# KrisKennaway/ii-vision

Hardware: AMD Instinct MI355X
Metric: DHGR frames transcoded/sec (higher is better)
Workload: dtype u16; 1 GPU; DHGR NTSC palette 560x192 S-iid synthetic clips, 750 frames each, 14336 independent clips per GPU, Movie.encode control flow (490 opcodes/frame, bank flip per 2 KiB); palette=NTSC, streams_per_gpu=14336, greedy_form=shared, resident_clip_frames=750, opcodes_per_frame=490, parallelism=1 GPU x 14336 independent streams, no collective

## Files before the change

### ii-vision_amd/csrc/iiv_prologue.hip

```cpp
#include "iiv_host.h"
#include "iiv_edit.h"
#include "iiv_stream.h"
#include "iiv_wave.h"

namespace iiv {


constexpr int kProThreads = 1024;

__device__ static inline void lds_barrier()
{
    asm volatile("s_waitcnt lgkmcnt(0)\n\ts_barrier" ::: "memory");
}

#ifdef IIV_STAMPS
#define IIV_STAMP(i)                                                        \
    do {                                                                    \
        __syncthreads();                                                    \
        if (threadIdx.x == 0) S.stamps[i] = __builtin_amdgcn_s_memtime();   \
    } while (0)
#else
#define IIV_STAMP(i) do { } while (0)
#endif

__device__ static inline void cmpx(unsigned long long &lo, unsigned long long &hi, bool asc)
{
    bool sw = (lo > hi) == asc;
    unsigned long long t = lo;
    lo = sw ? hi : lo;
    hi = sw ? t : hi;
}

template <int KPT, int NT>
__device__ static inline void bitonic_sort(unsigned long long (&v)[KPT], unsigned long long *xbuf, int tid)
{
    constexpr int N = KPT * NT;
#pragma unroll
    for (int k = 2; k <= KPT; k <<= 1) {
#pragma unroll
        for (int j = k >> 1; j >= 1; j >>= 1) {
#pragma unroll
            for (int r = 0; r < KPT; r++)
                if ((r & j) == 0) cmpx(v[r], v[r | j], (((KPT * tid + r) & k) == 0));
        }
    }
    for (int k = 2 * KPT; k <= N; k <<= 1) {
        const bool asc = ((KPT * tid) & k) == 0;
        for (int j = k >> 1; j >= KPT; j >>= 1) {
            const int d = j / KPT;
            const bool take_min = ((tid & d) == 0) == asc;
            if (d < 64) {
#pragma unroll
                for (int r = 0; r < KPT; r++) {
                    unsigned long long p = __shfl_xor(v[r], d, 64);
                    v[r] = take_min ? (p < v[r] ? p : v[r]) : (p > v[r] ? p : v[r]);
                }
            } else {
#pragma unroll
                for (int r = 0; r < KPT; r++) xbuf[r * NT + tid] = v[r];
                __syncthreads();
#pragma unroll
                for (int r = 0; r < KPT; r++) {
                    unsigned long long p = xbuf[r * NT + (tid ^ d)];
                    v[r] = take_min ? (p < v[r] ? p : v[r]) : (p > v[r] ? p : v[r]);
                }
                __syncthreads();
            }
        }
#pragma unroll
        for (int j = KPT >> 1; j >= 1; j >>= 1) {
#pragma unroll
            for (int r = 0; r < KPT; r++)
                if ((r & j) == 0) cmpx(v[r], v[r | j], asc);
        }
    }
}

template <int KPT> __device__ static inline void write_order(uint32_t *order, const unsigned long long (&v)[KPT], int tid)
{
    uint32_t o[KPT];
#pragma unroll
    for (int j = 0; j < KPT; j++) o[j] = ((uint32_t)(v[j] >> 8) & 0x1fffu) | (((uint32_t)v[j] & 0xffu) << 16);
    if (KPT == 2) {
        *reinterpret_cast<uint2 *>(order + 2 * tid) = make_uint2(o[0], o[1]);
    } else {
        uint4 *q = reinterpret_cast<uint4 *>(order + KPT * tid);
#pragma unroll
        for (int j = 0; j < KPT / 4; j++) q[j] = make_uint4(o[4 * j], o[4 * j + 1], o[4 * j + 2], o[4 * j + 3]);
    }
}

__device__ static inline int wave_scan_incl(int v)
{
    v += __builtin_amdgcn_update_dpp(0, v, 0x111, 0xf, 0xf, false);
    v += __builtin_amdgcn_update_dpp(0, v, 0x112, 0xf, 0xf, false);
    v += __builtin_amdgcn_update_dpp(0, v, 0x114, 0xf, 0xf, false);
    v += __builtin_amdgcn_update_dpp(0, v, 0x118, 0xf, 0xf, false);
    v += __builtin_amdgcn_update_dpp(0, v, 0x142, 0xa, 0xf, false);
    v += __builtin_amdgcn_update_dpp(0, v, 0x143, 0xc, 0xf, false);
    return v;
}

template <int NT> __device__ static inline int block_scan_excl(int v, int tid, uint32_t *wsum, int &total)
{
    static_assert(NT == 1024, "sixteen waves: their totals are scanned in one DPP row");
    const int incl = wave_scan_incl(v);
    lds_barrier();
    if ((tid & 63) == 63) wsum[tid >> 6] = (uint32_t)incl;
    lds_barrier();
    int x = (int)wsum[tid & 15];
    x += __builtin_amdgcn_update_dpp(0, x, 0x111, 0xf, 0xf, false);
    x += __builtin_amdgcn_update_dpp(0, x, 0x112, 0xf, 0xf, false);
    x += __builtin_amdgcn_update_dpp(0, x, 0x114, 0xf, 0xf, false);
    x += __builtin_amdgcn_update_dpp(0, x, 0x118, 0xf, 0xf, false);
    const int w = __builtin_amdgcn_readfirstlane(tid >> 6);
    total = __builtin_amdgcn_readlane(x, 15);
    const int wbase = w ? __builtin_amdgcn_readlane(x, w - 1) : 0;
    return wbase + incl - v;
}

template <int NT> __device__ static inline int block_scan_excl_and_max(int v, int m, int tid, uint32_t *wsum, uint32_t *wmax, int &total, int &maxv)
{
    static_assert(NT == 1024, "sixteen waves");
    auto mx = [](int a, int b) { return a > b ? a : b; };
    const int incl = wave_scan_incl(v);
    m = mx(m, __builtin_amdgcn_update_dpp(0, m, 0xB1, 0xf, 0xf, false));
    m = mx(m, __builtin_amdgcn_update_dpp(0, m, 0x4E, 0xf, 0xf, false));
    m = mx(m, __builtin_amdgcn_update_dpp(0, m, 0x141, 0xf, 0xf, false));
    m = mx(m, __builtin_amdgcn_update_dpp(0, m, 0x140, 0xf, 0xf, false));
    m = mx(m, __builtin_amdgcn_update_dpp(0, m, 0x142, 0xf, 0xf, false));
    m = mx(m, __builtin_amdgcn_update_dpp(0, m, 0x143, 0xf, 0xf, false));
    lds_barrier();
    if ((tid & 63) == 63) {
        wsum[tid >> 6] = (uint32_t)incl;
        wmax[tid >> 6] = (uint32_t)m;
    }
    lds_barrier();
    int x = (int)wsum[tid & 15], y = (int)wmax[tid & 15];
    x += __builtin_amdgcn_update_dpp(0, x, 0x111, 0xf, 0xf, false);
    x += __builtin_amdgcn_update_dpp(0, x, 0x112, 0xf, 0xf, false);
    x += __builtin_amdgcn_update_dpp(0, x, 0x114, 0xf, 0xf, false);
    x += __builtin_amdgcn_update_dpp(0, x, 0x118, 0xf, 0xf, false);
    y = mx(y, __builtin_amdgcn_update_dpp(0, y, 0xB1, 0xf, 0xf, false));
    y = mx(y, __builtin_amdgcn_update_dpp(0, y, 0x4E, 0xf, 0xf, false));
    y = mx(y, __builtin_amdgcn_update_dpp(0, y, 0x141, 0xf, 0xf, false));
    y = mx(y, __builtin_amdgcn_update_dpp(0, y, 0x140, 0xf, 0xf, false));
    const int w = __builtin_amdgcn_readfirstlane(tid >> 6);
    total = __builtin_amdgcn_readlane(x, 15);
    maxv = __builtin_amdgcn_readfirstlane(y);
    const int wbase = w ? __builtin_amdgcn_readlane(x, w - 1) : 0;
    return wbase + incl - v;
}

template <int NT> __device__ static inline int block_max(int v, int tid, uint32_t *wsum)
{
    static_assert(NT == 1024, "sixteen waves");
    auto mx = [](int a, int b) { return a > b ? a : b; };
    v = mx(v, __builtin_amdgcn_update_dpp(0, v, 0xB1, 0xf, 0xf, false));
    v = mx(v, __builtin_amdgcn_update_dpp(0, v, 0x4E, 0xf, 0xf, false));
    v = mx(v, __builtin_amdgcn_update_dpp(0, v, 0x141, 0xf, 0xf, false));
    v = mx(v, __builtin_amdgcn_update_dpp(0, v, 0x140, 0xf, 0xf, false));
    v = mx(v, __builtin_amdgcn_update_dpp(0, v, 0x142, 0xf, 0xf, false));
    v = mx(v, __builtin_amdgcn_update_dpp(0, v, 0x143, 0xf, 0xf, false));
    lds_barrier();
    if ((tid & 63) == 63) wsum[tid >> 6] = (uint32_t)v;
    lds_barrier();
    int x = (int)wsum[tid & 15];
    x = mx(x, __builtin_amdgcn_update_dpp(0, x, 0xB1, 0xf, 0xf, false));
    x = mx(x, __builtin_amdgcn_update_dpp(0, x, 0x4E, 0xf, 0xf, false));
    x = mx(x, __builtin_amdgcn_update_dpp(0, x, 0x141, 0xf, 0xf, false));
    x = mx(x, __builtin_amdgcn_update_dpp(0, x, 0x140, 0xf, 0xf, false));
    return __builtin_amdgcn_readfirstlane(x);
}

__device__ static inline bool any_half_is_big(const uint32_t (&w)[4])
{
    typedef unsigned short u16x2 __attribute__((ext_vector_type(2)));
    const u16x2 a = __builtin_elementwise_max(__builtin_bit_cast(u16x2, w[0]), __builtin_bit_cast(u16x2, w[1]));
    const u16x2 b = __builtin_elementwise_max(__builtin_bit_cast(u16x2, w[2]), __builtin_bit_cast(u16x2, w[3]));
    const uint32_t m = __builtin_bit_cast(uint32_t, __builtin_elementwise_max(a, b));
    return m >= 0xffff0000u || (m & 0xffffu) == kUpBig;
}

template <int MODE, int DP>
__device__ __forceinline__ void prologue_body(StreamState *__restrict__ states, const uint8_t *__restrict__ frames_main,
                                              const uint8_t *__restrict__ frames_aux, int n_frames, const LaunchSeg &seg,
                                              const uint16_t *__restrict__ table, const ulonglong2 *__restrict__ strings,
                                              const uint16_t *__restrict__ sub, const uint32_t *__restrict__ dwl,
                                              const uint32_t *__restrict__ dwr, const uint32_t *__restrict__ hgr_dots,
                                              const uint32_t *__restrict__ dw_pieces)
{
    const int need = __builtin_amdgcn_readfirstlane(seg.need);
    if (need < 0) return;
    const int frame = __builtin_amdgcn_readfirstlane(seg.frame), is_aux = __builtin_amdgcn_readfirstlane(seg.is_aux);
    constexpr int BITS = ModeTraits<MODE>::kBits;
    constexpr int NB = ModeTraits<MODE>::kBanks;
    __shared__ __attribute__((aligned(16))) unsigned char lds[9728 + 65536];
    uint32_t *aux4k = reinterpret_cast<uint32_t *>(lds + 512);
    uint32_t(*mtb)[624] = reinterpret_cast<uint32_t(*)[624]>(lds + 4608);
    uint32_t *wsum = reinterpret_cast<uint32_t *>(lds + 9600);
    int &flag_bad = *reinterpret_cast<int *>(lds + 9664);
    int &sel_bucket = *reinterpret_cast<int *>(lds + 9668);
    int &sel_count = *reinterpret_cast<int *>(lds + 9672);
    int &big_bucket = *reinterpret_cast<int *>(lds + 9676);
    unsigned char *smem = lds + 9728;
    unsigned long long *keys = reinterpret_cast<unsigned long long *>(smem);
    uint32_t *gen = reinterpret_cast<uint32_t *>(smem + 32768);

    const int tid = threadIdx.x;
    StreamState &S = states[blockIdx.x];
    const size_t fbase = ((size_t)blockIdx.x * n_frames + frame) * 8192;

    IIV_STAMP(0);
    const int first = S.mt_np_idx;
    const int error_in = S.error;
    if (tid == 0) flag_bad = 0;
    uint32_t *gtab = reinterpret_cast<uint32_t *>(smem);
    uint32_t *hdot = aux4k;
    if (DP == IIV_DW_RECURRENCE) {
        reinterpret_cast<uint4 *>(gtab)[tid] = reinterpret_cast<const uint4 *>(dw_pieces + (MODE == kDHGR ? 4096 * is_aux : 0))[tid];
        if (MODE == kHGR) {
            constexpr int kRest = (int)kHgrPieceWords / 4 - kProThreads;
            static_assert(kRest > 0 && kRest <= kProThreads && kHgrPieceWords * 4 <= 32768, "the HGR pair-term table ends below the generated MT19937 blocks");
            if (tid < kRest) reinterpret_cast<uint4 *>(gtab)[kProThreads + tid] = reinterpret_cast<const uint4 *>(dw_pieces)[kProThreads + tid];
            if (tid >= kProThreads - kHgrDotLutEntries / 4) {
                const int q = tid - (kProThreads - kHgrDotLutEntries / 4);
                reinterpret_cast<uint4 *>(hdot)[q] = reinterpret_cast<const uint4 *>(hgr_dots)[q];
            }
        }
    }
    IIV_STAMP(10);
    for (int i = tid; i < 624; i += kProThreads) mtb[0][i] = S.mt_np[i];
    IIV_STAMP(11);
    __syncthreads();
    IIV_STAMP(1);
    const int own_b = (MODE == kDHGR && is_aux) ? 1 : 0;
    const int tgt_first = tid == 0 ? (int)((own_b ? frames_aux : frames_main) + fbase)[0] : 0;
    const int i0 = tid * 8;
    const bool mt_wave = tid >= kProThreads - 64;
    uint16_t *dwx = reinterpret_cast<uint16_t *>(mtb[1]);

    int32_t upv[8];
    {
        const uint4 a = *reinterpret_cast<const uint4 *>(S.up16[is_aux] + i0);
        const uint32_t w[4] = {a.x, a.y, a.z, a.w};
#pragma unroll
        for (int j = 0; j < 4; j++) {
            upv[2 * j] = (int32_t)(w[j] & 0xffffu);
            upv[2 * j + 1] = (int32_t)(w[j] >> 16);
        }
        if (any_half_is_big(w)) {
#pragma unroll
            for (int j = 0; j < 8; j++)
                if ((uint32_t)upv[j] == kUpBig) upv[j] = S.up[is_aux][i0 + j];
        }
    }
    if (mt_wave) {
        __builtin_amdgcn_s_setprio(3);
        const uint32_t *src = mtb[0];
#ifndef IIV_EXP_MT_BLOCKS
#define IIV_EXP_MT_BLOCKS 13
#endif
        const int n_blocks = __builtin_amdgcn_readfirstlane((first + 7679) / 624);
        const int nb = n_blocks < IIV_EXP_MT_BLOCKS ? n_blocks : IIV_EXP_MT_BLOCKS;
#ifndef IIV_HGR_MT_REGISTERS
#define IIV_HGR_MT_REGISTERS 1
#endif
        if (MODE == kDHGR || IIV_HGR_MT_REGISTERS) {
            mt_generate_wave(src, gen, nb, tid & 63);
        } else {
            for (int k = 0; k < nb; k++) {
                mt_twist_wave(src, gen + k * 624, tid & 63);
                src = gen + k * 624;
            }
        }
        __builtin_amdgcn_s_setprio(0);
    }
    IIV_STAMP(12);

    auto diff_weight = [&](uint32_t cm, uint32_t tm, int y) -> uint32_t {
        const int odd = y & 1;
        const int o = byte_offset<MODE>(y, is_aux);
        if (DP == IIV_DW_TABLE) return table[((size_t)o << (2 * BITS)) + ((size_t)cm << BITS) + tm];
        if (DP == IIV_DW_SPLIT) {
            using T = SplitTraits<MODE>;
            const uint32_t l = dwl[((((uint32_t)o << T::kLeftRowBits) + split_row_left<MODE>(cm, odd)) << T::kLeftRowBits) +
                                   split_row_left<MODE>(tm, odd)];
            const uint32_t r = dwr[((((uint32_t)o << T::kRightRowBits) + split_row_right<MODE>(cm, odd)) << T::kRightRowBits) +
                                   split_row_right<MODE>(tm, odd)];
            return combine(l, r);
        }
        if constexpr (MODE == kDHGR) {
            return 0u;
        } else {
            return hgr_dw_pieces_sum(hdot, reinterpret_cast<const unsigned char *>(gtab), cm, tm, odd);
        }
    };

    uint32_t dwv[8], tmv[8];
    uint32_t cpk[2] = {0, 0};
    int bad = 0;
    {
        const bool hole = is_hole(i0 & 255);
        const bool proxy = hole && !mt_wave;
        int grp = tid;
        if (proxy) {
            const int k = tid >> 4;
            grp = 960 + k + k / 15;
        }
        const int yb = (grp * 8) & 255;
#pragma unroll
        for (int j = 0; j < 8; j++) tmv[j] = dwv[j] = 0;
        const int oth_b = NB - 1 - own_b;
        const uint8_t *cur_own_g = S.mem[own_b] + grp * 8, *cur_oth_g = S.mem[oth_b] + grp * 8;
        const uint8_t *tgt_own_g = (own_b ? frames_aux : frames_main) + fbase + grp * 8;
        const uint8_t *tgt_oth_g = (oth_b ? frames_aux : frames_main) + fbase + grp * 8;
        unsigned long long own8[2], prv8[2], nxt8[2];
#pragma unroll
        for (int k = 0; k < 2; k++) {
            const uint8_t *own = k ? tgt_own_g : cur_own_g, *oth = k ? tgt_oth_g : cur_oth_g;
            own8[k] = *reinterpret_cast<const unsigned long long *>(own);
            if (MODE != kDHGR) {
                const unsigned long long before = yb > 0 ? own[-1] : 0, after = yb + 8 < 256 ? own[8] : 0;
                prv8[k] = (own8[k] << 8) | before;
                nxt8[k] = (own8[k] >> 8) | (after << 56);
                continue;
            }
            const unsigned long long o8 = *reinterpret_cast<const unsigned long long *>(oth);
            if (is_aux) {
                const unsigned long long before = yb > 0 ? oth[-1] : 0;
                prv8[k] = (o8 << 8) | before;
                nxt8[k] = o8;
            } else {
                const unsigned long long after = yb + 8 < 256 ? oth[8] : 0;
                prv8[k] = o8;
                nxt8[k] = (o8 >> 8) | (after << 56);
            }
        }
        if (hole) {
            const unsigned long long mine = proxy ? *reinterpret_cast<const unsigned long long *>(S.mem[own_b] + i0) : own8[0];
            if (mine) bad = kErrHoles;
        }
        if (!proxy) {
            cpk[0] = (uint32_t)own8[1];
            cpk[1] = (uint32_t)(own8[1] >> 32);
        }
        auto dw_pieces_sum = [&](uint32_t W, int parity) -> uint32_t {
            uint32_t acc = 0;
#pragma unroll
            for (int i = 0; i < 5; i++) {
                const uint32_t cur6 = __builtin_amdgcn_ubfe(W, 16 + 2 * i, 6);
                const uint32_t tgt6x4 = (i == 0 ? W << 2 : i == 1 ? W : W >> (2 * i - 2)) & 0xfcu;
                const uint32_t v = *reinterpret_cast<const uint32_t *>(reinterpret_cast<const unsigned char *>(gtab) + ((cur6 << 8) | tgt6x4));
                acc += ((i + parity) & 1) ? v >> 16 : v & 0xffffu;
            }
            return acc - 5u * kDwPieceBias;
        };
        if (!hole || proxy) {
#pragma unroll
            for (int j = 0; j < 8; j++) {
                const int jj = j & 3;
                const uint32_t sel = 0x0c000c00u | (uint32_t)jj | ((uint32_t)(4 + jj) << 16);
                auto pick = [&](const unsigned long long (&v)[2]) -> uint32_t {
                    const uint32_t c = j < 4 ? (uint32_t)v[0] : (uint32_t)(v[0] >> 32), t = j < 4 ? (uint32_t)v[1] : (uint32_t)(v[1] >> 32);
                    return __builtin_amdgcn_perm(c, t, sel);
                };
                const uint32_t pb = pick(prv8), ob = pick(own8), nb = pick(nxt8);
                if constexpr (MODE == kDHGR) {
                    const uint32_t W = ((pb >> 3) & 0x000e000eu) | ((ob & 0x007f007fu) << 4) | ((nb & 0x00070007u) << 11);
                    if (!proxy) tmv[j] = (W >> 1) & 0x1fffu;
                    if (!mt_wave) {
                        uint32_t d;
                        if (DP == IIV_DW_RECURRENCE) d = dw_pieces_sum(W, j & 1);
                        else d = diff_weight(W >> 17, (W >> 1) & 0x1fffu, yb + j);
                        if (proxy) dwx[(grp - 960) * 8 + j] = (uint16_t)d;
                        else dwv[j] = d;
                    }
                } else {
                    const uint32_t mid = (j & 1) ? ((ob & 0x007f007fu) << 4) | ((ob & 0x00800080u) >> 4) : ob << 3;
                    const uint32_t W = ((pb >> 5) & 0x00070007u) | mid | ((nb & 0x00030003u) << 12) | ((nb & 0x00800080u) << 4);
                    if (!proxy) tmv[j] = W & 0x3fffu;
                    if (!mt_wave) {
                        const uint32_t d = diff_weight(W >> 16, W & 0x3fffu, yb + j);
                        if (proxy) dwx[(grp - 960) * 8 + j] = (uint16_t)d;
                        else dwv[j] = d;
                    }
                }
            }
        }
    }
    uint32_t nzmask = 0;
    auto finish_bytes = [&]() {
#pragma unroll
        for (int j = 0; j < 8; j++) {
            int32_t u = upv[j];
            if (dwv[j] == 0) u = 0;
            u += (int32_t)dwv[j];
            if (u < 0) bad = kErrNegative;
            upv[j] = u;
            if (u != 0) nzmask |= 1u << j;
        }
        uint32_t pk[4];
#pragma unroll
        for (int j = 0; j < 4; j++) {
            typedef unsigned short u16x2 __attribute__((ext_vector_type(2)));
            const u16x2 c = __builtin_amdgcn_cvt_pk_u16((uint32_t)upv[2 * j], (uint32_t)upv[2 * j + 1]);
            pk[j] = __builtin_bit_cast(uint32_t, c);
        }
        *reinterpret_cast<uint4 *>(S.up16[is_aux] + i0) = make_uint4(pk[0], pk[1], pk[2], pk[3]);
        if (any_half_is_big(pk)) {
#pragma unroll
            for (int j = 0; j < 8; j++)
                if ((uint32_t)upv[j] >= kUpBig) S.up[is_aux][i0 + j] = upv[j];
        }
        uint4 *q = reinterpret_cast<uint4 *>(S.wd + i0);
        uint32_t wv[8];
#pragma unroll
        for (int j = 0; j < 8; j++)
            wv[j] = wd_word(split_row_left<MODE>(tmv[j], j & 1), split_row_right<MODE>(tmv[j], j & 1), dwv[j]);
        q[0] = make_uint4(wv[0], wv[1], wv[2], wv[3]);
        q[1] = make_uint4(wv[4], wv[5], wv[6], wv[7]);
        reinterpret_cast<uint8_t *>(S.nzbits)[tid] = (uint8_t)nzmask;
    };
    constexpr bool kFinishEarly = true;
    if (error_in) return;
    if (kFinishEarly && !mt_wave) finish_bytes();
    __builtin_amdgcn_s_setprio(3);
    lds_barrier();
    if (mt_wave && !is_hole(i0 & 255)) {
#pragma unroll
        for (int j = 0; j < 8; j++) dwv[j] = dwx[(tid - (kProThreads - 64)) * 8 + j];
    }
    if (!kFinishEarly || mt_wave) finish_bytes();
    if (tid < 256) S.pdone[tid] = 0;
    if (bad) flag_bad = bad;

    IIV_STAMP(2);
    uint32_t *hist = aux4k;
    uint32_t *wmax = reinterpret_cast<uint32_t *>(mtb[1]);
    uint16_t *start = reinterpret_cast<uint16_t *>(mtb[1]) + 64;
    int n, sh;
    int mx = 0;
#pragma unroll
    for (int j = 0; j < 8; j++) mx = upv[j] > mx ? upv[j] : mx;
    hist[tid] = 0;
    const int rank0 = block_scan_excl_and_max<kProThreads>(__popc(nzmask), mx, tid, wsum, wmax, n, mx);
    sh = mx < 1024 ? 0 : (32 - __clz(mx)) - 10;
    if (tid == 0) {
        sel_bucket = 0;
        sel_count = n;
        big_bucket = 0;
    }
#pragma unroll
    for (int j = 0; j < 8; j++)
        if (nzmask & (1u << j)) atomicAdd(&hist[upv[j] >> sh], 1u);
    lds_barrier();
    const int bcount = (int)hist[1023 - tid];
    int total_unused;
    const int bstart = block_scan_excl<kProThreads>(bcount, tid, wsum, total_unused);
    const bool want_prefix = need > 0 && need <= kSelNeedMax && n > need;
    if (want_prefix && bstart < need && bstart + bcount >= need) {
        sel_bucket = 1023 - tid;
        sel_count = bstart + bcount;
    }
    lds_barrier();
    const int n_sel = sel_count;
    const int first_bucket = sel_bucket;
    if (bcount > kBucketMax && (1023 - tid) >= first_bucket) big_bucket = 1;
    uint32_t selmask = 0;
#pragma unroll
    for (int j = 0; j < 8; j++)
        if ((nzmask & (1u << j)) && (upv[j] >> sh) >= first_bucket) selmask |= 1u << j;
    lds_barrier();
    const bool by_buckets = big_bucket == 0;
    uint32_t *cursor = aux4k;
    cursor[1023 - tid] = (uint32_t)bstart;
    start[1023 - tid] = (uint16_t)bstart;

    IIV_STAMP(3);
    if (!flag_bad) {
        const int blk = first + n > 0 ? (first + n - 1) / 624 : 0;
        const uint32_t *fin = blk ? gen + (blk - 1) * 624 : mtb[0];
        for (int w = tid; w < 624; w += kProThreads) S.mt_np[w] = fin[w];
        if (tid == 0) {
            S.mt_np_idx = first + n - blk * 624;
            S.draws_np += (unsigned long long)n;
        }
    }

    IIV_STAMP(4);
    unsigned long long kv[8];
    {
        int bk = (first + rank0) / 624, bw = first + rank0 - bk * 624;
#pragma unroll
        for (int j = 0; j < 8; j++) {
            kv[j] = ~0ull;
            if (nzmask & (1u << j)) {
                if (selmask & (1u << j)) {
                    const uint32_t nonce = mt_temper((bk ? gen + (bk - 1) * 624 : mtb[0])[bw]) & 0xffu;
                    kv[j] = ((unsigned long long)(0x7fffffffu - (uint32_t)upv[j]) << 29) |
                            ((unsigned long long)nonce << 21) | ((unsigned long long)(i0 + j) << 8) |
                            (unsigned long long)((cpk[j >> 2] >> (8 * (j & 3))) & 0xffu);
                }
                if (++bw == 624) {
                    bw = 0;
                    bk++;
                }
            }
        }
    }
    IIV_STAMP(5);
    if (by_buckets) {
        lds_barrier();
        IIV_STAMP(8);
        uint32_t slot[8];
#pragma unroll
        for (int j = 0; j < 8; j++) {
            slot[j] = 0;
            if (kv[j] != ~0ull) slot[j] = atomicAdd(&cursor[(0x7fffffffu - (uint32_t)(kv[j] >> 29)) >> sh], 1u);
        }
#pragma unroll
        for (int j = 0; j < 8; j++)
            if (kv[j] != ~0ull) keys[slot[j]] = kv[j];
        lds_barrier();
        IIV_STAMP(9);
        for (int t = tid; t < n_sel; t += kProThreads) {
            const unsigned long long key = keys[t];
            const int bk = (int)((0x7fffffffu - (uint32_t)(key >> 29)) >> sh);
            const int s0 = (int)start[bk];
            const int e0 = bk == 0 ? n : (int)start[bk - 1];
            const int last = e0 - 1;
            int below = 0;
            int i = s0;
            for (; i + 16 <= e0; i += 16) {
                unsigned long long kk[16];
#pragma unroll
                for (int u = 0; u < 16; u++) kk[u] = keys[i + u];
#pragma unroll
                for (int u = 0; u < 16; u++) below += kk[u] < key ? 1 : 0;
            }
            for (; i < e0; i += 4) {
                const unsigned long long k0 = keys[i];
                const unsigned long long k1 = keys[i + 1 < e0 ? i + 1 : last];
                const unsigned long long k2 = keys[i + 2 < e0 ? i + 2 : last];
                const unsigned long long k3 = keys[i + 3 < e0 ? i + 3 : last];
                below += (k0 < key ? 1 : 0) + ((i + 1 < e0 && k1 < key) ? 1 : 0) +
                         ((i + 2 < e0 && k2 < key) ? 1 : 0) + ((i + 3 < e0 && k3 < key) ? 1 : 0);
            }
            S.order[s0 + below] = ((uint32_t)(key >> 8) & 0x1fffu) | (((uint32_t)key & 0xffu) << 16);
        }
    } else if (n_sel <= 4 * kProThreads) {
        __syncthreads();
        int tot;
        int nsel_mine = 0;
#pragma unroll
        for (int j = 0; j < 8; j++) nsel_mine += kv[j] != ~0ull ? 1 : 0;
        int pos = block_scan_excl<kProThreads>(nsel_mine, tid, wsum, tot);
        const bool small = tot <= 2 * kProThreads;
        const int n_pad = small ? 2 * kProThreads : 4 * kProThreads;
        for (int i = tot + tid; i < n_pad; i += kProThreads) keys[i] = ~0ull;
#pragma unroll
        for (int j = 0; j < 8; j++)
            if (kv[j] != ~0ull) keys[pos++] = kv[j];
        __syncthreads();
        if (small) {
            unsigned long long v2[2] = {keys[2 * tid], keys[2 * tid + 1]};
            __syncthreads();
            bitonic_sort<2, kProThreads>(v2, keys, tid);
            write_order<2>(S.order, v2, tid);
        } else {
            unsigned long long v4[4] = {keys[4 * tid], keys[4 * tid + 1], keys[4 * tid + 2], keys[4 * tid + 3]};
            __syncthreads();
            bitonic_sort<4, kProThreads>(v4, keys, tid);
            write_order<4>(S.order, v4, tid);
        }
    } else {
        __syncthreads();
        bitonic_sort<8, kProThreads>(kv, keys, tid);
        write_order<8>(S.order, kv, tid);
    }
    IIV_STAMP(6);
    IIV_STAMP(7);
    if (tid == 0) {
        S.n_sorted = n_sel;
        S.truncated = n_sel < n ? 1 : 0;
        S.head = 0;
        S.n_pushed = 0;
        S.exhausted = 0;
        S.gen_active = 1;
        S.gen_is_aux = is_aux;
        S.gen_frame = frame;
        S.pad_content = tgt_first;
        if (flag_bad && S.error == 0) S.error = flag_bad;
    }
}

template <int MODE, int DP>
__global__ __launch_bounds__(kProThreads, 8) void prologue_kernel(StreamState *__restrict__ states,
                                                               const uint8_t *__restrict__ frames_main,
                                                               const uint8_t *__restrict__ frames_aux, int n_frames,
                                                               const LaunchSeg *__restrict__ segs, int seg_stride,
                                                               const uint16_t *__restrict__ table,
                                                               const ulonglong2 *__restrict__ strings,
                                                               const uint16_t *__restrict__ sub,
                                                               const uint32_t *__restrict__ dwl,
                                                               const uint32_t *__restrict__ dwr,
                                                               const uint32_t *__restrict__ hgr_dots,
                                                               const uint32_t *__restrict__ dw_pieces)
{
    const LaunchSeg seg = segs[(size_t)blockIdx.x * seg_stride];
    prologue_body<MODE, DP>(states, frames_main, frames_aux, n_frames, seg, table, strings, sub, dwl, dwr, hgr_dots, dw_pieces);
}

int launch_prologue(int mode, int dw_mode, const PrologueArgs &a, hipStream_t st)
{
#define IIV_PRO(M, D)                                                                                                    \
    hipLaunchKernelGGL((prologue_kernel<M, D>), dim3(a.n_streams), dim3(kProThreads), 0, st, a.states, a.frames_main,     \
                       a.frames_aux, a.n_frames, a.segs, a.seg_stride, a.table, a.strings, a.sub, a.dwl, a.dwr, a.hgr_dots, a.dw_pieces)
    if (mode == kDHGR) {
        if (dw_mode == IIV_DW_SPLIT) IIV_PRO(kDHGR, IIV_DW_SPLIT);
        else if (dw_mode == IIV_DW_RECURRENCE) IIV_PRO(kDHGR, IIV_DW_RECURRENCE);
        else IIV_PRO(kDHGR, IIV_DW_TABLE);
    } else {
        if (dw_mode == IIV_DW_SPLIT) IIV_PRO(kHGR, IIV_DW_SPLIT);
        else if (dw_mode == IIV_DW_RECURRENCE) IIV_PRO(kHGR, IIV_DW_RECURRENCE);
        else IIV_PRO(kHGR, IIV_DW_TABLE);
    }
#undef IIV_PRO
    return hip_check(hipGetLastError(), "prologue_kernel launch");
}

}
```

### ii-vision_amd/csrc/iiv_stream.h

```cpp
#pragma once

#include "iiv_device.h"
#include "iiv_edit.h"

#include <type_traits>

namespace iiv {

constexpr int kPushedCap = 24576;

constexpr int kWdDwShift = 20;
constexpr int kWdDwBits = 12;
constexpr int kWdRightShift = 12, kWdLeftShift = 22;
__host__ __device__ inline uint32_t wd_word(uint32_t row_left, uint32_t row_right, uint32_t dw)
{
    return (row_left << (kWdLeftShift + 1)) | (row_right << (kWdRightShift + 1)) | ((0u - dw) & ((1u << kWdDwBits) - 1u));
}
__host__ __device__ inline uint32_t wd_dw(uint32_t wd) { return (0u - wd) & ((1u << kWdDwBits) - 1u); }
__host__ __device__ inline uint32_t wd_off_left(uint32_t wd) { return wd >> kWdLeftShift; }
__host__ __device__ inline uint32_t wd_off_right(uint32_t wd) { return (wd >> kWdRightShift) & 0x3ffu; }
constexpr uint32_t kDwPieceBias = 512;
constexpr uint32_t kHgrPieceStride = 67;
constexpr uint32_t kHgrPieceWords = 4288;
__device__ __forceinline__ uint32_t hgr_dw_pieces_sum(const uint32_t *__restrict__ dots, const unsigned char *__restrict__ g, uint32_t cm, uint32_t tm, int odd)
{
    const uint32_t Dc = dots[hgr_dot_slot_lo(cm, odd)] | dots[hgr_dot_slot_hi(cm, odd)];
    const uint32_t Dt = dots[hgr_dot_slot_lo(tm, odd)] | dots[hgr_dot_slot_hi(tm, odd)];
    uint32_t acc = 0;
#pragma unroll
    for (int i = 0; i < 9; i++) {
        const uint32_t cur6 = __builtin_amdgcn_ubfe(Dc, 2 * i, 6);
        const uint32_t tgt6x4 = (i == 0 ? Dt << 2 : i == 1 ? Dt : Dt >> (2 * i - 2)) & 0xfcu;
        acc += *reinterpret_cast<const uint16_t *>(g + (__umul24(cur6, 4u * kHgrPieceStride) + tgt6x4) + 2 * ((i & 1) ^ odd));
    }
    return acc - 9u * kDwPieceBias;
}
constexpr int kMaxValue = 2047;

struct StreamState {
    uint8_t mem[2][8192];
    int32_t up[2][8192];
    uint32_t wd[8192];
    uint32_t order[8192];
    uint32_t nzbits[256];
    uint32_t pdone[256];
    uint32_t pushed[kPushedCap];
    uint32_t mt_py[624];
    uint32_t mt_np[624];
    int32_t mt_py_idx, mt_np_idx;
    int32_t n_sorted, head, n_pushed, exhausted;
    int32_t gen_active, gen_is_aux, gen_frame, error;
    int32_t out_of_work[2];
    int32_t pad_content;
    int32_t truncated;
    unsigned long long draws_py, draws_np, ops, pad_ops;
    unsigned long long stat_exact, stat_ops, stat_runs;
    unsigned long long stamps[32];
    uint16_t up16[2][8192];
};
constexpr uint32_t kUpBig = 0xffffu;
__device__ inline int32_t up_value(const StreamState &S, int b, int i)
{
    const uint32_t v = S.up16[b][i];
    return v == kUpBig ? S.up[b][i] : (int32_t)v;
}

enum { kErrNone = 0, kErrHoles = 1, kErrNegative = 2, kErrPaletteBit = 3, kErrPushedOverflow = 4, kErrNoGenerator = 5, kErrGuard = 6, kErrSortBudget = 7, kErrBankMix = 8 };

struct LaunchSeg {
    int32_t frame;
    int32_t is_aux;
    int32_t n_ops;
    int32_t ops_base;
    int32_t need;
};

template <int MODE> struct SplitTraits;
template <> struct SplitTraits<kDHGR> {
    static constexpr int kCut = 5, kLeftRowBits = 8, kRightRowBits = 9, kLeftCBits = 5, kRightCBits = 6;
};
template <> struct SplitTraits<kHGR> {
    static constexpr int kCut = 9, kLeftRowBits = 9, kRightRowBits = 9, kLeftCBits = 6, kRightCBits = 6;
};

template <int MODE> __host__ __device__ constexpr uint32_t split_mask_left(int o)
{
    return MODE == kDHGR ? 0x00ffu : ((o & 1) ? 0x01ffu : 0x04ffu);
}
template <int MODE> __host__ __device__ constexpr uint32_t split_mask_right(int o)
{
    return MODE == kDHGR ? 0x1ff0u : ((o & 1) ? 0x3fc8u : 0x3fe0u);
}
template <int MODE> __host__ __device__ constexpr uint32_t split_mask_own() { return MODE == kDHGR ? 0x7fu << 3 : 0xffu << 3; }

template <int MODE> __host__ __device__ inline uint32_t split_row_left(uint32_t win, int odd)
{
    if (MODE == kDHGR) return win & 0xffu;
    return odd ? (win & 0x1ffu) : ((win & 0xffu) | (((win >> 10) & 1u) << 8));
}
template <int MODE> __host__ __device__ inline uint32_t split_row_right(uint32_t win, int odd)
{
    if (MODE == kDHGR) return win >> 4;
    return odd ? (((win >> 3) & 1u) | ((win >> 6) << 1)) : (win >> 5);
}
template <int MODE> __host__ __device__ inline uint32_t split_content_left(uint32_t c, int odd)
{
    if (MODE == kDHGR) return c & 31u;
    const uint32_t rc = ((c & 0x7fu) << 1) | (c >> 7);
    return odd ? (rc & 63u) : ((c & 31u) | ((c >> 7) << 5));
}
template <int MODE> __host__ __device__ inline uint32_t split_content_right(uint32_t c, int odd)
{
    if (MODE == kDHGR) return (c >> 1) & 63u;
    const uint32_t rc = ((c & 0x7fu) << 1) | (c >> 7);
    return odd ? ((rc & 1u) | ((rc >> 3) << 1)) : (c >> 2);
}
template <int MODE> __host__ __device__ constexpr size_t split_left_entries()
{
    return (size_t)ModeTraits<MODE>::kOffsets << (SplitTraits<MODE>::kLeftCBits + SplitTraits<MODE>::kLeftRowBits);
}
template <int MODE> __host__ __device__ constexpr size_t split_right_entries()
{
    return (size_t)ModeTraits<MODE>::kOffsets << (SplitTraits<MODE>::kRightCBits + SplitTraits<MODE>::kRightRowBits);
}
template <int MODE> __host__ __device__ constexpr size_t split_dw_left_entries()
{
    return (size_t)ModeTraits<MODE>::kOffsets << (2 * SplitTraits<MODE>::kLeftRowBits);
}
template <int MODE> __host__ __device__ constexpr size_t split_dw_right_entries()
{
    return (size_t)ModeTraits<MODE>::kOffsets << (2 * SplitTraits<MODE>::kRightRowBits);
}
constexpr uint32_t kSplitInf = 0x3fffu;

__host__ __device__ inline uint32_t split_combine(uint32_t l, uint32_t r)
{
    const uint32_t a = (l & 0xffffu) + (r & 0xffffu), b = (l >> 16) + (r >> 16);
    return a < b ? a : b;
}

constexpr uint32_t kNarrowBias = 256;
struct NarrowTables {
    const uint8_t *base;
    uint32_t right_off;
    int exact;
};
template <int MODE> __host__ __device__ constexpr uint32_t narrow_right_off() { return (uint32_t)split_left_entries<MODE>() * 2; }
template <int MODE> __host__ __device__ constexpr size_t narrow_total_bytes()
{
    return narrow_right_off<MODE>() + split_right_entries<MODE>() * 2;
}
template <int MODE> struct JointPack {
    static constexpr int kPairs = (1 << ModeTraits<MODE>::kContentBits) / 128;
};
template <int MODE> __host__ __device__ constexpr size_t joint_left_entries()
{
    return ((size_t)ModeTraits<MODE>::kOffsets << SplitTraits<MODE>::kLeftRowBits) * JointPack<MODE>::kPairs * 64;
}
template <int MODE> __host__ __device__ constexpr size_t joint_right_entries()
{
    return ((size_t)ModeTraits<MODE>::kOffsets << SplitTraits<MODE>::kRightRowBits) * JointPack<MODE>::kPairs * 64;
}
template <int MODE> __host__ __device__ inline uint32_t split_window_from_rows(uint32_t row_left, uint32_t row_right, int odd)
{
    if (MODE == kDHGR) return (row_right << 4) | (row_left & 15u);
    return odd ? ((row_right >> 1) << 6) | (row_left & 63u) : (row_right << 5) | (row_left & 31u);
}

__device__ static inline void wave_lds_sync()
{
    __builtin_amdgcn_fence(__ATOMIC_RELEASE, "wavefront");
    __builtin_amdgcn_wave_barrier();
    __builtin_amdgcn_fence(__ATOMIC_ACQUIRE, "wavefront");
}

__device__ static inline void mt_twist_wave(const uint32_t *__restrict__ src, uint32_t *__restrict__ dst, int lane)
{
    auto mt_mix = [](uint32_t x, uint32_t y) -> uint32_t {
        const uint32_t v = (x & 0x80000000u) | (y & 0x7fffffffu);
        return (v >> 1) ^ ((uint32_t)__builtin_amdgcn_sbfe(y, 0, 1) & 0x9908b0dfu);
    };
    uint32_t a[4], b[4], c[3];
#pragma unroll
    for (int g = 0; g < 4; g++) {
        const int j = lane + 64 * g;
        a[g] = b[g] = 0;
        if (g < 3 || j < 227) {
            a[g] = src[j + 397] ^ mt_mix(src[j], src[j + 1]);
            b[g] = a[g] ^ mt_mix(src[227 + j], src[228 + j]);
        }
    }
    const uint32_t new0 = (uint32_t)__builtin_amdgcn_readlane((int)a[0], 0);
#pragma unroll
    for (int g = 0; g < 3; g++) {
        const int j = lane + 64 * g;
        c[g] = 0;
        if (g < 2 || j < 170) {
            const uint32_t nx = (g == 2 && j == 169) ? new0 : src[(g == 2 && j == 169) ? 0 : 455 + j];
            c[g] = b[g] ^ mt_mix(src[454 + j], nx);
        }
    }
#pragma unroll
    for (int g = 0; g < 4; g++) {
        const int j = lane + 64 * g;
        if (g < 3 || j < 227) {
            dst[j] = a[g];
            dst[227 + j] = b[g];
        }
        if (g < 2 || (g == 2 && j < 170)) dst[454 + j] = c[g];
    }
    wave_lds_sync();
}

struct MtRegs {
    uint32_t A[4], B[4], C[3];
};
struct MtLaneConsts {
    int addr7, addr42;
    bool lt22, lt57;
    __device__ explicit MtLaneConsts(int lane) : addr7(((lane + 7) & 63) << 2), addr42(((lane + 42) & 63) << 2), lt22(lane < 22), lt57(lane < 57) {}
};
__device__ static inline void mt_regs_load(MtRegs &m, const uint32_t *__restrict__ blk, int lane)
{
#pragma unroll
    for (int g = 0; g < 4; g++) {
        const int j = lane + 64 * g;
        m.A[g] = m.B[g] = 0;
        if (g < 3 || j < 227) {
            m.A[g] = blk[j];
            m.B[g] = blk[227 + j];
        }
        if (g < 3) {
            m.C[g] = 0;
            if (g < 2 || j < 170) m.C[g] = blk[454 + j];
        }
    }
}
__device__ static inline void mt_regs_store(const MtRegs &m, uint32_t *__restrict__ dst, int lane)
{
#pragma unroll
    for (int g = 0; g < 4; g++) {
        const int j = lane + 64 * g;
        if (g < 3 || j < 227) {
            dst[j] = m.A[g];
            dst[227 + j] = m.B[g];
        }
        if (g < 2 || (g == 2 && j < 170)) dst[454 + j] = m.C[g];
    }
}
__device__ __forceinline__ void mt_regs_twist(MtRegs &m, const MtLaneConsts &k)
{
    auto mix = [](uint32_t x, uint32_t y) -> uint32_t {
        const uint32_t v = (x & 0x80000000u) | (y & 0x7fffffffu);
        return (v >> 1) ^ ((uint32_t)__builtin_amdgcn_sbfe(y, 0, 1) & 0x9908b0dfu);
    };
    auto up1 = [&](uint32_t v, uint32_t next0, auto last) -> uint32_t {
        uint32_t s = (uint32_t)__builtin_amdgcn_update_dpp(0, (int)v, 0x130, 0xf, 0xf, false);
        asm("v_writelane_b32 %0, %1, %2" : "+v"(s) : "s"(next0), "n"(decltype(last)::value));
        return s;
    };
    auto lane0 = [](uint32_t v) -> uint32_t { return (uint32_t)__builtin_amdgcn_readlane((int)v, 0); };
    auto rot = [](uint32_t v, int addr) -> uint32_t { return (uint32_t)__builtin_amdgcn_ds_bpermute(addr, (int)v); };
    uint32_t(&A)[4] = m.A, (&B)[4] = m.B, (&C)[3] = m.C;
    const uint32_t rb2 = rot(B[2], k.addr42), rb3 = rot(B[3], k.addr42);
    const uint32_t rc0 = rot(C[0], k.addr7), rc1 = rot(C[1], k.addr7), rc2 = rot(C[2], k.addr7);
    uint32_t X[4];
    X[0] = k.lt22 ? rb2 : k.lt57 ? rb3 : rc0;
    X[1] = k.lt57 ? rc0 : rc1;
    X[2] = k.lt57 ? rc1 : rc2;
    X[3] = rc2;
    uint32_t nA[4], nB[4], nC[3];
#pragma unroll
    for (int g = 0; g < 4; g++)
        nA[g] = X[g] ^ mix(A[g], g < 3 ? up1(A[g], lane0(A[g < 3 ? g + 1 : 0]), std::integral_constant<int, 63>{}) : up1(A[g], lane0(B[0]), std::integral_constant<int, 34>{}));
#pragma unroll
    for (int g = 0; g < 4; g++)
        nB[g] = nA[g] ^ mix(B[g], g < 3 ? up1(B[g], lane0(B[g < 3 ? g + 1 : 0]), std::integral_constant<int, 63>{}) : up1(B[g], lane0(C[0]), std::integral_constant<int, 34>{}));
#pragma unroll
    for (int g = 0; g < 3; g++)
        nC[g] = nB[g] ^ mix(C[g], g < 2 ? up1(C[g], lane0(C[g < 2 ? g + 1 : 0]), std::integral_constant<int, 63>{}) : up1(C[g], lane0(nA[0]), std::integral_constant<int, 41>{}));
#pragma unroll
    for (int g = 0; g < 4; g++) {
        A[g] = nA[g];
        B[g] = nB[g];
        if (g < 3) C[g] = nC[g];
    }
}
__device__ static inline uint32_t mt_regs_gather(const MtRegs &m, int idx, int lo, int hi)
{
    auto code_of = [](int i, int &j) -> int {
        const int t = (i >= 227 ? 1 : 0) + (i >= 454 ? 1 : 0);
        j = i - 227 * t;
        return 4 * t + (j >> 6);
    };
    int j, jl, jh;
    const int code = code_of(idx, j);
    const int c_lo = code_of(lo, jl), c_hi = code_of(hi, jh);
    const int addr = (j & 63) << 2;
    uint32_t r = 0;
#pragma unroll
    for (int k = 0; k < 11; k++) {
        if (k >= c_lo && k <= c_hi) {
            const uint32_t src = k < 4 ? m.A[k] : k < 8 ? m.B[k - 4] : m.C[k - 8];
            const uint32_t v = (uint32_t)__builtin_amdgcn_ds_bpermute(addr, (int)src);
            r = code == k ? v : r;
        }
    }
    return r;
}

__device__ static inline void mt_generate_wave(const uint32_t *__restrict__ blk0, uint32_t *__restrict__ gen, int n_blocks, int lane)
{
    MtRegs m;
    mt_regs_load(m, blk0, lane);
    const MtLaneConsts kc(lane);
    for (int k = 0; k < n_blocks; k++) {
        mt_regs_twist(m, kc);
        mt_regs_store(m, gen + k * 624, lane);
    }
    wave_lds_sync();
}

struct GreedyArgs {
    StreamState *states;
    const uint8_t *frames_main, *frames_aux;
    int n_frames, n_streams;
    const LaunchSeg *segs;
    int seg_stride;
    const uint32_t *left, *right;
    NarrowTables nt;
    uint8_t *ops_out;
    size_t ops_stride;
    int lds_pad;
    int uniform_bank;
    bool shared;
    int *queue;
    bool fourth;
    bool count_stats;
    const int *perm;
    uint32_t *cost;
    unsigned long long *live = nullptr;
    uint32_t live_tag = 0;
};

int launch_greedy_wave(int mode, const GreedyArgs &a, hipStream_t st, int *form_out = nullptr);
int launch_greedy_team(int mode, const GreedyArgs &a, hipStream_t st);


constexpr int kSelNeedMax = 2048;
constexpr int kBucketMax = 384;
struct PrologueArgs {
    StreamState *states;
    const uint8_t *frames_main, *frames_aux;
    int n_frames, n_streams;
    const LaunchSeg *segs;
    int seg_stride;
    const uint16_t *table;
    const ulonglong2 *strings;
    const uint16_t *sub;
    const uint32_t *dwl, *dwr;
    const uint32_t *hgr_dots;
    const uint32_t *dw_pieces;
};
int launch_prologue(int mode, int dw_mode, const PrologueArgs &a, hipStream_t st);
struct WorkgroupArgs {
    StreamState *states;
    const uint8_t *frames_main, *frames_aux;
    int n_frames, n_streams;
    const LaunchSeg *segs;
    int seg_stride;
    const uint16_t *store;
    const uint32_t *left_t, *right_t;
    uint8_t *ops_out;
    size_t ops_stride;
};
int launch_greedy_workgroup(int mode, int joint, bool fourth, const WorkgroupArgs &a, hipStream_t st);

}
```

Baseline: 3.450 million frames/s.

## Remap prologue threads so the MT wave owns the screen holes

Reassigns the 1024 prologue threads so the last wave, which generates the Mersenne Twister blocks, owns the 64 screen-hole groups. The other 960 threads own exactly the 960 visible groups. This removes the proxy path, in which non-MT threads computed diff weights for the MT wave's groups and passed them through LDS, along with the post-barrier finish_bytes pass the MT wave ran on that data. The MT wave now only checks that its holes are zero and writes constant zero/default words. The risk is that dropping wave_lds_sync and the HGR non-register MT path changes ordering or HGR behaviour.

Result: no change. 3.536 million frames/s (median of 3 runs) (+2.5%).

```diff
diff --git a/ii-vision_amd/csrc/iiv_prologue.hip b/ii-vision_amd/csrc/iiv_prologue.hip
--- a/ii-vision_amd/csrc/iiv_prologue.hip
+++ b/ii-vision_amd/csrc/iiv_prologue.hip
@@ -236,12 +236,38 @@
     IIV_STAMP(1);
     const int own_b = (MODE == kDHGR && is_aux) ? 1 : 0;
     const int tgt_first = tid == 0 ? (int)((own_b ? frames_aux : frames_main) + fbase)[0] : 0;
-    const int i0 = tid * 8;
-    const bool mt_wave = tid >= kProThreads - 64;
-    uint16_t *dwx = reinterpret_cast<uint16_t *>(mtb[1]);
+    const bool mt_wave = __builtin_amdgcn_readfirstlane(tid >> 6) == kProThreads / 64 - 1;
+    int grp;
+    if (mt_wave) {
+        const int k = tid - (kProThreads - 64);
+        grp = (k >> 1) * 32 + 15 + 16 * (k & 1);
+    } else {
+        const int row = tid / 30, c = tid - row * 30;
+        grp = row * 32 + c + (c >= 15 ? 1 : 0);
+    }
+    const int i0 = grp * 8;
+#ifndef IIV_EXP_MT_BLOCKS
+#define IIV_EXP_MT_BLOCKS 13
+#endif
 
     int32_t upv[8];
-    {
+    int bad = 0;
+    if (mt_wave) {
+        __builtin_amdgcn_s_setprio(3);
+        const unsigned long long mine = *reinterpret_cast<const unsigned long long *>(S.mem[own_b] + i0);
+        const int n_blocks = __builtin_amdgcn_readfirstlane((first + 7679) / 624);
+        const int nb = n_blocks < IIV_EXP_MT_BLOCKS ? n_blocks : IIV_EXP_MT_BLOCKS;
+        MtRegs mt;
+        const MtLaneConsts kc(tid & 63);
+        mt_regs_load(mt, mtb[0], tid & 63);
+        for (int k = 0; k < nb; k++) {
+            mt_regs_twist(mt, kc);
+            mt_regs_store(mt, gen + k * 624, tid & 63);
+        }
+        if (mine) bad = kErrHoles;
+#pragma unroll
+        for (int j = 0; j < 8; j++) upv[j] = 0;
+    } else {
         const uint4 a = *reinterpret_cast<const uint4 *>(S.up16[is_aux] + i0);
         const uint32_t w[4] = {a.x, a.y, a.z, a.w};
 #pragma unroll
@@ -254,27 +280,6 @@
             for (int j = 0; j < 8; j++)
                 if ((uint32_t)upv[j] == kUpBig) upv[j] = S.up[is_aux][i0 + j];
         }
-    }
-    if (mt_wave) {
-        __builtin_amdgcn_s_setprio(3);
-        const uint32_t *src = mtb[0];
-#ifndef IIV_EXP_MT_BLOCKS
-#define IIV_EXP_MT_BLOCKS 13
-#endif
-        const int n_blocks = __builtin_amdgcn_readfirstlane((first + 7679) / 624);
-        const int nb = n_blocks < IIV_EXP_MT_BLOCKS ? n_blocks : IIV_EXP_MT_BLOCKS;
-#ifndef IIV_HGR_MT_REGISTERS
-#define IIV_HGR_MT_REGISTERS 1
-#endif
-        if (MODE == kDHGR || IIV_HGR_MT_REGISTERS) {
-            mt_generate_wave(src, gen, nb, tid & 63);
-        } else {
-            for (int k = 0; k < nb; k++) {
-                mt_twist_wave(src, gen + k * 624, tid & 63);
-                src = gen + k * 624;
-            }
-        }
-        __builtin_amdgcn_s_setprio(0);
     }
     IIV_STAMP(12);
 
@@ -299,22 +304,12 @@
 
     uint32_t dwv[8], tmv[8];
     uint32_t cpk[2] = {0, 0};
-    int bad = 0;
-    {
-        const bool hole = is_hole(i0 & 255);
-        const bool proxy = hole && !mt_wave;
-        int grp = tid;
-        if (proxy) {
-            const int k = tid >> 4;
-            grp = 960 + k + k / 15;
-        }
-        const int yb = (grp * 8) & 255;
-#pragma unroll
-        for (int j = 0; j < 8; j++) tmv[j] = dwv[j] = 0;
+    if (!mt_wave) {
+        const int yb = i0 & 255;
         const int oth_b = NB - 1 - own_b;
-        const uint8_t *cur_own_g = S.mem[own_b] + grp * 8, *cur_oth_g = S.mem[oth_b] + grp * 8;
-        const uint8_t *tgt_own_g = (own_b ? frames_aux : frames_main) + fbase + grp * 8;
-        const uint8_t *tgt_oth_g = (oth_b ? frames_aux : frames_main) + fbase + grp * 8;
+        const uint8_t *cur_own_g = S.mem[own_b] + i0, *cur_oth_g = S.mem[oth_b] + i0;
+        const uint8_t *tgt_own_g = (own_b ? frames_aux : frames_main) + fbase + i0;
+        const uint8_t *tgt_oth_g = (oth_b ? frames_aux : frames_main) + fbase + i0;
         unsigned long long own8[2], prv8[2], nxt8[2];
 #pragma unroll
         for (int k = 0; k < 2; k++) {
@@ -337,14 +332,8 @@
                 nxt8[k] = (o8 >> 8) | (after << 56);
             }
         }
-        if (hole) {
-            const unsigned long long mine = proxy ? *reinterpret_cast<const unsigned long long *>(S.mem[own_b] + i0) : own8[0];
-            if (mine) bad = kErrHoles;
-        }
-        if (!proxy) {
-            cpk[0] = (uint32_t)own8[1];
-            cpk[1] = (uint32_t)(own8[1] >> 32);
-        }
+        cpk[0] = (uint32_t)own8[1];
+        cpk[1] = (uint32_t)(own8[1] >> 32);
         auto dw_pieces_sum = [&](uint32_t W, int parity) -> uint32_t {
             uint32_t acc = 0;
 #pragma unroll
@@ -356,36 +345,25 @@
             }
             return acc - 5u * kDwPieceBias;
         };
-        if (!hole || proxy) {
-#pragma unroll
-            for (int j = 0; j < 8; j++) {
-                const int jj = j & 3;
-                const uint32_t sel = 0x0c000c00u | (uint32_t)jj | ((uint32_t)(4 + jj) << 16);
-                auto pick = [&](const unsigned long long (&v)[2]) -> uint32_t {
-                    const uint32_t c = j < 4 ? (uint32_t)v[0] : (uint32_t)(v[0] >> 32), t = j < 4 ? (uint32_t)v[1] : (uint32_t)(v[1] >> 32);
-                    return __builtin_amdgcn_perm(c, t, sel);
-                };
-                const uint32_t pb = pick(prv8), ob = pick(own8), nb = pick(nxt8);
-                if constexpr (MODE == kDHGR) {
-                    const uint32_t W = ((pb >> 3) & 0x000e000eu) | ((ob & 0x007f007fu) << 4) | ((nb & 0x00070007u) << 11);
-                    if (!proxy) tmv[j] = (W >> 1) & 0x1fffu;
-                    if (!mt_wave) {
-                        uint32_t d;
-                        if (DP == IIV_DW_RECURRENCE) d = dw_pieces_sum(W, j & 1);
-                        else d = diff_weight(W >> 17, (W >> 1) & 0x1fffu, yb + j);
-                        if (proxy) dwx[(grp - 960) * 8 + j] = (uint16_t)d;
-                        else dwv[j] = d;
-                    }
-                } else {
-                    const uint32_t mid = (j & 1) ? ((ob & 0x007f007fu) << 4) | ((ob & 0x00800080u) >> 4) : ob << 3;
-                    const uint32_t W = ((pb >> 5) & 0x00070007u) | mid | ((nb & 0x00030003u) << 12) | ((nb & 0x00800080u) << 4);
-                    if (!proxy) tmv[j] = W & 0x3fffu;
-                    if (!mt_wave) {
-                        const uint32_t d = diff_weight(W >> 16, W & 0x3fffu, yb + j);
-                        if (proxy) dwx[(grp - 960) * 8 + j] = (uint16_t)d;
-                        else dwv[j] = d;
-                    }
-                }
+#pragma unroll
+        for (int j = 0; j < 8; j++) {
+            const int jj = j & 3;
+            const uint32_t sel = 0x0c000c00u | (uint32_t)jj | ((uint32_t)(4 + jj) << 16);
+            auto pick = [&](const unsigned long long (&v)[2]) -> uint32_t {
+                const uint32_t c = j < 4 ? (uint32_t)v[0] : (uint32_t)(v[0] >> 32), t = j < 4 ? (uint32_t)v[1] : (uint32_t)(v[1] >> 32);
+                return __builtin_amdgcn_perm(c, t, sel);
+            };
+            const uint32_t pb = pick(prv8), ob = pick(own8), nb = pick(nxt8);
+            if constexpr (MODE == kDHGR) {
+                const uint32_t W = ((pb >> 3) & 0x000e000eu) | ((ob & 0x007f007fu) << 4) | ((nb & 0x00070007u) << 11);
+                tmv[j] = (W >> 1) & 0x1fffu;
+                if (DP == IIV_DW_RECURRENCE) dwv[j] = dw_pieces_sum(W, j & 1);
+                else dwv[j] = diff_weight(W >> 17, (W >> 1) & 0x1fffu, yb + j);
+            } else {
+                const uint32_t mid = (j & 1) ? ((ob & 0x007f007fu) << 4) | ((ob & 0x00800080u) >> 4) : ob << 3;
+                const uint32_t W = ((pb >> 5) & 0x00070007u) | mid | ((nb & 0x00030003u) << 12) | ((nb & 0x00800080u) << 4);
+                tmv[j] = W & 0x3fffu;
+                dwv[j] = diff_weight(W >> 16, W & 0x3fffu, yb + j);
             }
         }
     }
@@ -420,18 +398,21 @@
             wv[j] = wd_word(split_row_left<MODE>(tmv[j], j & 1), split_row_right<MODE>(tmv[j], j & 1), dwv[j]);
         q[0] = make_uint4(wv[0], wv[1], wv[2], wv[3]);
         q[1] = make_uint4(wv[4], wv[5], wv[6], wv[7]);
-        reinterpret_cast<uint8_t *>(S.nzbits)[tid] = (uint8_t)nzmask;
+        reinterpret_cast<uint8_t *>(S.nzbits)[grp] = (uint8_t)nzmask;
     };
-    constexpr bool kFinishEarly = true;
     if (error_in) return;
-    if (kFinishEarly && !mt_wave) finish_bytes();
+    if (!mt_wave) {
+        finish_bytes();
+    } else {
+        *reinterpret_cast<uint4 *>(S.up16[is_aux] + i0) = make_uint4(0, 0, 0, 0);
+        const uint32_t w0 = wd_word(split_row_left<MODE>(0, 0), split_row_right<MODE>(0, 0), 0);
+        const uint32_t w1 = wd_word(split_row_left<MODE>(0, 1), split_row_right<MODE>(0, 1), 0);
+        uint4 *q = reinterpret_cast<uint4 *>(S.wd + i0);
+        q[0] = q[1] = make_uint4(w0, w1, w0, w1);
+        reinterpret_cast<uint8_t *>(S.nzbits)[grp] = 0;
+    }
     __builtin_amdgcn_s_setprio(3);
     lds_barrier();
-    if (mt_wave && !is_hole(i0 & 255)) {
-#pragma unroll
-        for (int j = 0; j < 8; j++) dwv[j] = dwx[(tid - (kProThreads - 64)) * 8 + j];
-    }
-    if (!kFinishEarly || mt_wave) finish_bytes();
     if (tid < 256) S.pdone[tid] = 0;
     if (bad) flag_bad = bad;
 
diff --git a/ii-vision_amd/csrc/iiv_stream.h b/ii-vision_amd/csrc/iiv_stream.h
--- a/ii-vision_amd/csrc/iiv_stream.h
+++ b/ii-vision_amd/csrc/iiv_stream.h
@@ -309,18 +309,6 @@
     return r;
 }
 
-__device__ static inline void mt_generate_wave(const uint32_t *__restrict__ blk0, uint32_t *__restrict__ gen, int n_blocks, int lane)
-{
-    MtRegs m;
-    mt_regs_load(m, blk0, lane);
-    const MtLaneConsts kc(lane);
-    for (int k = 0; k < n_blocks; k++) {
-        mt_regs_twist(m, kc);
-        mt_regs_store(m, gen + k * 624, lane);
-    }
-    wave_lds_sync();
-}
-
 struct GreedyArgs {
     StreamState *states;
     const uint8_t *frames_main, *frames_aux;
```
